# MadrMan/gpgpuraytrace

Measured on AMD Instinct MI355X. Metric: Mray/s + ms/frame at 1920×1080, 1/2/4/8 MI355X; % HBM roofline, higher is better.
Workload: dtype f32

## Files before the change

### gpgpuraytrace_amd/csrc/rt_kernels.hip

```cpp
#include <hip/hip_runtime.h>

#include <cstdio>
#include <cstdlib>
#include <type_traits>

#include "rt_kernels.h"
#include "rt_shader.h"
#include "rt_variants.h"

using namespace rts;
using rtm::f3;

namespace {

constexpr int kPermWords = 128 * 128;
constexpr int kNpOct = RT_NP_OCTAVES + 3;
constexpr int kOctWords = kNpOct * 4;
constexpr int kOctBase = (int)kLdsGz / 4 + (int)(kLdsGz - kLdsGxy) / 4;
constexpr int kNoiseLdsWords = kOctBase + kOctWords;
static_assert(kNoiseLdsWords % 4 == 0, "LDS carved after the noise image stays 16-byte aligned");
static_assert(kLdsGxy == (uint32_t)kPermWords * 4u, "gxy follows the perm2D texels");

__device__ __forceinline__ void load_noise_lds(uint32_t* lds, const uint32_t* __restrict__ perm2d,
                                               const float4* __restrict__ grad, const RtConsts* __restrict__ k)
// ... 100 lines not shown

template <bool STATS, int BS, int LPR>
__global__ void __launch_bounds__(BS) k_camerarays_group(const RtConsts* __restrict__ k,
                                                          const uint32_t* __restrict__ perm2d,
                                                          const float4* __restrict__ grad, float4* __restrict__ out,
                                                          RtStats* stats, const FrameTable* __restrict__ ft)
{
    constexpr int L = RT_NOMADPLAINS;
    if (ft) out = ft->cam[blockIdx.y];
    __shared__ __attribute__((aligned(16))) uint32_t lds[kNoiseLdsWords];
    load_noise_lds(lds, perm2d, grad, k);
    const int i = blockIdx.x * (BS / LPR) + (int)(threadIdx.x / LPR);
    if (i >= RT_CAMERA_RES * RT_CAMERA_RES) return;
    Ctx c = make_ctx(k, lds);
    if (ft) c = frame_ctx_cam(c, ft, blockIdx.y);
    const uint32_t j = threadIdx.x & (LPR - 1u), base = threadIdx.x & 63u & ~(LPR - 1u);
    const SegOctaves<LPR> g = seg_octaves<LPR>(c, j);
    int tx = i % RT_CAMERA_RES, ty = i / RT_CAMERA_RES;
    const float r31 = rtm::rcp(31.0f);
    uint32_t pxs = (uint32_t)(((float)tx * r31) * k->screen[0]);
    uint32_t pys = (uint32_t)(((float)ty * r31) * k->screen[1]);
    f3 p, dir;
    get_pixel_ray(c, (float)pxs, (float)pys, &p, &dir);
    March<L, false> st;
    march_begin(c, st, p, RT_CAMERA_NEAR, 2.0f, dir);
    uint32_t noise = 0;
    while (march_live<L, false, true>(c, st, RT_CAMERA_FAR, 0)) {
        auto dens = [&](f3 q) {
            uint32_t used;
            float d = density_nomadplains_seg<LPR>(c, g, q, j, base, &used);
            noise += used + 1u;
            return d;
        };
        march_step_with<L, false, true, decltype(dens), true>(c, st, dens);
    }
    RayResult rr = march_result(st);
    if (rr.density < 0.0f) rr.pd.w = RT_CAMERA_FAR;
    if (j == 0) {
        out[i] = make_float4(rr.pd.x, rr.pd.y, rr.pd.z, rr.pd.w);
        if constexpr (STATS) {
            atomicAdd(&stats->prepass_steps, (unsigned long long)rr.steps);
            atomicAdd(&stats->noise_calls, (unsigned long long)noise);
        }
    }
}

template <class Depth>
__device__ __forceinline__ float cd_get_depth(Depth depth, int x, int y)
{
    x = x < 0 ? 0 : (x >= RT_CAMERA_RES ? RT_CAMERA_RES - 1 : x);
    y = y < 0 ? 0 : (y >= RT_CAMERA_RES ? RT_CAMERA_RES - 1 : y);
    return depth(x, y);
}
template <class Depth>
__device__ __forceinline__ float cd_interp(Depth d, int x, int y)
{
    if (x < 0) {
        float m = cd_get_depth(d, x + 1, y);
        float dd = cd_get_depth(d, x + 2, y) - m;
        return m - dd;
    }
    if (x >= RT_CAMERA_RES) {
        float m = cd_get_depth(d, x - 1, y);
        float dd = cd_get_depth(d, x - 2, y) - m;
        return m - dd;
    }
    if (y < 0) {
// ... 980 lines not shown
                live = true;
            }
            __builtin_amdgcn_s_waitcnt(0);
            if (lane == 0) {
                q.l_head = head + take;
                q.ls_top = sl - more;
            }
            q_unlock(&q.lock, lane);
            const uint32_t lid = late(lane);
            const uint32_t j = lid & (LPR - 1u), base = lid & ~(LPR - 1u);
            const SegOctaves<LPR> g = seg_octaves<LPR>(c, j);
            for (;;) {
                if (live && !march_live<L, true, true>(cl, st, aux_ao(aux) ? RT_AO_END : 100.0f, 0)) {
                    if (j == 0u) {
                        stat(aux_ao(aux) ? BlockStats::AO : BlockStats::SHADOW, (uint32_t)st.iters);
                        if (kAoSlots > 0u && aux_ao_slot(aux)) ao_slot_finish(st, t, aux);
                        else long_finish<L>(k, m, s_fr, fin, finp, samples, aocc, t, aux, st);
                    }
                    live = false;
                }
                if (!__ballot(live)) break;
                WT(wt[25]++;)
                if (live) {
                    auto dens = [&](f3 q0) {
                        uint32_t used;
                        const float d = density_nomadplains_seg<LPR>(cl, g, q0, j, base, &used);
                        if constexpr (STATS) {
                            if (j == 0u) atomicAdd(&s_st.v[BlockStats::NOISE], (unsigned long long)(used + 1u));
                            if (lane == (uint32_t)__builtin_ctzll(__ballot(1)))
                                atomicAdd(&s_st.v[BlockStats::NOISE_WAVES], (unsigned long long)SegOctaves<LPR>::R);
                        }
                        return d;
                    };
                    march_step_with<L, true, true, decltype(dens), true>(cl, st, dens);
                }
            }
            uint32_t fa = j == 0u ? aux : kAuxAO;
            if (__ballot(fa < kFinSlots || aux_slot_free(fa))) {
                q_lock(&q.lock, lane);
                free_fin_locked(false, fa);
                q_unlock(&q.lock, lane);
            }
        }
    };

    auto primary_seg = [&](const Ctx& cf, March<L, true>& st, bool lv, uint64_t lb, float spx, float spy) {
        if constexpr (L == RT_NOMADPLAINS && kPrimarySeg > 0u && (!STATS || kStatsPrimarySeg)) {
            constexpr uint32_t LPR = 64u / (kPrimarySeg ? kPrimarySeg : 8u);
            const uint32_t lid = late(lane);
            const uint32_t j = lid & (LPR - 1u), grp = lid / LPR, base = lid & ~(LPR - 1u);
            const uint32_t n = (uint32_t)__popcll(lb);
            uint32_t src = lid;
            uint64_t rem = lb;
            for (uint32_t r = 0; r < n; ++r) {
                const uint32_t sl = (uint32_t)__builtin_ctzll(rem);
                rem &= rem - 1ull;
                src = grp == r ? sl : src;
            }
            March<L, true> sg;
            sg.p = rtm::mk(__shfl(st.p.x, (int)src), __shfl(st.p.y, (int)src), __shfl(st.p.z, (int)src));
            sg.dir = rtm::mk(__shfl(st.dir.x, (int)src), __shfl(st.dir.y, (int)src), __shfl(st.dir.z, (int)src));
            sg.sd = __shfl(st.sd, (int)src);
            sg.dist = __shfl(st.dist, (int)src);
            sg.step = __shfl(st.step, (int)src);
            sg.lastStep = __shfl(st.lastStep, (int)src);
            sg.d = __shfl(st.d, (int)src);
            sg.iters = __shfl(st.iters, (int)src);
            sg.f = {0.0f, 0.0f, 0.0f, 0.0f};
            sg.fog = false;
            bool live = grp < n;
            const SegOctaves<LPR> g = seg_octaves<LPR>(cf, j);
            for (;;) {
                if (live && !march_live<L, true, false>(cf, sg, RT_CAMERA_FAR, max_steps)) live = false;
                if (!__ballot(live)) break;
                if (live) {
                    auto dens = [&](f3 q0) {
                        uint32_t used;
                        const float d = density_nomadplains_seg<LPR, true>(cf, g, q0, j, base, &used);
                        if constexpr (STATS) {
                            if (j == 0u) atomicAdd(&s_st.v[BlockStats::NOISE], (unsigned long long)(used + 1u));
                            if (lane == (uint32_t)__builtin_ctzll(__ballot(1)))
                                atomicAdd(&s_st.v[BlockStats::NOISE_WAVES], (unsigned long long)SegOctaves<LPR>::R);
                        }
                        return d;
                    };
                    march_step_with<L, true, false, decltype(dens), true>(cf, sg, dens);
                }
            }
            const int back = (int)(lane_rank(lb) * LPR);
            const float sd = __shfl(sg.sd, back), dist = __shfl(sg.dist, back), step = __shfl(sg.step, back);
            const float last = __shfl(sg.lastStep, back), d = __shfl(sg.d, back);
            const int iters = __shfl(sg.iters, back);
            if (lv) {
                st.sd = sd;
                st.dist = dist;
                st.step = step;
                st.lastStep = last;
                st.d = d;
                st.iters = iters;
            }
            f3 p, dir;
            get_pixel_ray(cf, spx, spy, &p, &dir);
            st.p = p;
            st.dir = rtm::scale(dir, rtm::rcp(rtm::length(dir)));
        }
    };

    auto do_shade = [&]() {
        q_lock(&q.lock, lane);
        const uint32_t top = vload(q.h_top);
        const uint32_t take = top < 64u ? top : 64u;
        float4 r0 = make_float4(0.0f, 0.0f, 0.0f, 0.0f), r1 = r0, r2 = r0;
        if (lane < take) {
            const uint32_t ri = (top - take + lane) * HR;
            r0 = ld_rec(hq, ri);
            if constexpr (HR == 3u) {
                r1 = ld_rec(hq, ri + 1u);
                r2 = ld_rec(hq, ri + 2u);
            }
// ... 78 lines not shown
            push_long(valid, ao, t, ao_aux);
        }
    };

    auto do_prepass = [&](const FrameTable* __restrict__ pft, uint32_t qt, bool own) {
        if constexpr (L == RT_NOMADPLAINS) {
            constexpr uint32_t LPR = RT_PREPASS_LPR, RPW = 64u / LPR;
            constexpr uint32_t WPF = RT_CAMERA_RES * RT_CAMERA_RES / RPW;
            const uint32_t f = qt / WPF;
            const uint32_t ray0 = (qt - f * WPF) * RPW;
            const uint32_t ray = ray0 + late(lane) / LPR;
            const uint32_t lid = late(lane);
            const uint32_t j = lid & (LPR - 1u), base = lid & ~(LPR - 1u);
            Ctx cp = c;
            cp.k = pft->kcam[0];
            cp.kf = (KPtr)pft->kcam[f];
            cp.eye = rtm::mk(uniform_f(cp.kf->eye[0]), uniform_f(cp.kf->eye[1]), uniform_f(cp.kf->eye[2]));
            cp.sun = rtm::mk(uniform_f(cp.kf->sun[0]), uniform_f(cp.kf->sun[1]), uniform_f(cp.kf->sun[2]));
            const uint32_t tx = ray % RT_CAMERA_RES, ty = ray / RT_CAMERA_RES;
            const float r31 = rtm::rcp(31.0f);
            const uint32_t pxs = (uint32_t)(((float)tx * r31) * cp.k->screen[0]);
            const uint32_t pys = (uint32_t)(((float)ty * r31) * cp.k->screen[1]);
            f3 p, dir;
            get_pixel_ray(cp, (float)pxs, (float)pys, &p, &dir);
            March<L, false> st;
            march_begin(cp, st, p, RT_CAMERA_NEAR, 2.0f, dir);
            const SegOctaves<LPR> g = seg_octaves<LPR>(cp, j);
            __builtin_amdgcn_s_setprio(RT_FUSE_PRIO);
            while (march_live<L, false, true>(cp, st, RT_CAMERA_FAR, 0)) {
                auto dens = [&](f3 q0) {
                    uint32_t used;
                    return density_nomadplains_seg<LPR, false>(cp, g, q0, j, base, &used);
                };
                march_step_with<L, false, true, decltype(dens), true>(cp, st, dens);
            }
            __builtin_amdgcn_s_setprio(0);
            RayResult rr = march_result(st);
            if (rr.density < 0.0f) rr.pd.w = RT_CAMERA_FAR;
            if (j == 0u) {
                typedef float v4f __attribute__((ext_vector_type(4)));
                const v4f v = {rr.pd.x, rr.pd.y, rr.pd.z, rr.pd.w};
                float4* dst = pft->cam[f] + ray;
                asm volatile("global_store_dwordx4 %0, %1, off sc1" : : "v"(dst), "v"(v) : "memory");
            }
            asm volatile("s_waitcnt vmcnt(0)" : : : "memory");
            if (!own) {
                if (lane == 0) __hip_atomic_fetch_add(np.ctl + 1, RPW, __ATOMIC_RELAXED, __HIP_MEMORY_SCOPE_AGENT);
                return;
            }
            typedef uint32_t __attribute__((address_space(1))) guint;
            guint* gf = (guint*)(gp.gate + f * RT_GATE_WORDS);
            uint32_t old = 0;
            if (lane == 0) {
                const uint32_t task = ray0 / RT_FUSE_RAYS_PER_TASK;
                bool whole = true;
                if constexpr (RPW < RT_FUSE_RAYS_PER_TASK)
                    whole = __hip_atomic_fetch_add(gf + RT_GATE_TASKS + task, RPW, __ATOMIC_RELAXED,
                                                   __HIP_MEMORY_SCOPE_AGENT) == RT_FUSE_RAYS_PER_TASK - RPW;
                if (whole) {
                    __hip_atomic_fetch_or(gf + (task >> 5), 1u << (task & 31u), __ATOMIC_RELAXED, __HIP_MEMORY_SCOPE_AGENT);
                    old = __hip_atomic_fetch_add(gf + RT_GATE_CTR, (uint32_t)RT_FUSE_RAYS_PER_TASK, __ATOMIC_RELAXED,
                                                 __HIP_MEMORY_SCOPE_AGENT);
                }
            }
            if ((uint32_t)__builtin_amdgcn_readfirstlane(old) == RT_CAMERA_RES * RT_CAMERA_RES - RT_FUSE_RAYS_PER_TASK) {
                if (gp.debug & 2u) {
                    const uint64_t t0 = __builtin_amdgcn_s_memrealtime();
// ... 122 lines not shown
        }
        Ctx cf = frame_ctx(c, ft, f);
        cf.nz.phase = RT_PHASE_PRIMARY;
        uint32_t px, py;
        const bool valid = unit_pixel(m, f, u, lane, W, H, &px, &py);
        const float pxf = (float)px, pyf = (float)py;
        float plane_x = 0.0f;
        if (valid) {
            float spx = pxf * k->rcp_w, spy = pyf * k->rcp_h;
            const uint32_t cell = (uint32_t)rtm::fma(rtm::floor(spy * 32.0f), 32.0f, rtm::floor(spx * 32.0f));
            if (GATED && !cells_in) {
                const float4* cam = ft->cam[f];
                plane_x = cell_bracket([&](int x, int y) { return cam_depth_sc1(cam, x, y); }, (int)(cell % RT_CAMERA_RES),
                                       (int)(cell / RT_CAMERA_RES)).x;
            } else if (GATED) {
                typedef const float __attribute__((address_space(1))) gcfloat;
                plane_x = __hip_atomic_load((gcfloat*)(ft->cells[f] + cell), __ATOMIC_RELAXED, __HIP_MEMORY_SCOPE_AGENT);
            } else {
                plane_x = gptr(ft->cells[f])[cell].x;
            }
        }
        for (uint32_t a = 0; a < aa; ++a) {
            const uint32_t t = f * m.frame_samples + (u * 64u + lane) * aa + a;
            March<L, true> st;
            st.d = 0.0f;
            bool lv = false;
            if (valid) {
                f3 p, dir;
                get_pixel_ray(cf, pxf + k->aa_off[a][0], pyf + k->aa_off[a][1], &p, &dir);
                march_begin(cf, st, p, plane_x, 1.0f, dir);
                lv = true;
            }
            __builtin_amdgcn_s_setprio(0);
            for (uint32_t it = 0;; ++it) {
                lv = lv && march_live<L, true, false>(cf, st, RT_CAMERA_FAR, max_steps);
                const uint64_t lb = __ballot(lv);
                if (lb == 0ull) break;
                RT_DIAG_LIVE_HIST(if (lane == (uint32_t)__builtin_ctzll(__ballot(1))) atomicAdd(&g_live_hist[__popcll(lb)], 1ull);)
                RT_DIAG_PRIMARY_STEPS(if (lv) {
                    cf.nz.phase = RT_COUNT_PHASE;
                    count_noise(cf.nz);
                    cf.nz.phase = RT_PHASE_PRIMARY;
                })
                if constexpr (L == RT_NOMADPLAINS && kPrimarySeg > 0u && (!STATS || kStatsPrimarySeg)) {
                    if ((uint32_t)__popcll(lb) <= kPrimarySeg) {
                        primary_seg(cf, st, lv, lb, pxf + k->aa_off[a][0], pyf + k->aa_off[a][1]);
                        break;
                    }
                }
#if RT_FBM_EXIT
                if constexpr (L == RT_NOMADPLAINS) {
                    if (lv) {
                        const float ns = st.step * k->step_factor;
                        const bool allow = st.dist + ns < RT_CAMERA_FAR && ns > k->min_limit &&
                                           !(max_steps > 0 && st.iters + 1 >= max_steps);
                        march_step_with<L, true, false>(cf, st, [&](f3 q) { return density_nomadplains_x(cf, q, allow); });
                    }
                } else
#endif
                if (lv) march_step<L, true, false>(cf, st);
                if (it == 96u) __builtin_amdgcn_s_setprio(1);
                else if (it == 224u) __builtin_amdgcn_s_setprio(2);
                else if (it == 384u) __builtin_amdgcn_s_setprio(3);
            }
            __builtin_amdgcn_s_setprio(0);
            const bool hit = valid && st.d > 0.0f;
            WT(if (valid) wp_maxit = max(wp_maxit, (uint32_t)st.iters);)
            RayResult rr;
            if (valid) {
                rr = march_result(st);
                stat(BlockStats::PRIMARY, (uint32_t)st.iters);
                if (!hit) {
                    const float4 v = miss_sample(cf, pxf + k->aa_off[a][0], pyf + k->aa_off[a][1], rr.pd.w, rr.fc);
                    if (aa == 1u) {
                        const uint32_t px8 = unorm8(v.x) | (unorm8(v.y) << 8) | (unorm8(v.z) << 16) | 0xff000000u;
                        if (m.packed) {
                            if (!(RT_DIAG_SKIP & 1)) gptr(ft->out8[f])[packed_index(late(u * 64u + lane))] = px8;
                        } else {
                            const size_t o = (size_t)py * W + px;
                            if (!(RT_DIAG_SKIP & 1)) gptr(ft->out8[f])[o] = px8;
                            if (float4* o32 = ft->out32[f]) gstore(o32 + o, make_float4(v.x, v.y, v.z, 1.0f));
                        }
                    } else {
                        samples[t] = v;
                    }
                }
            }
            const uint64_t hb = __ballot(hit);
            if (lane == 0) hitmask[(f * m.n_units + u) * aa + a] = (m.fit || m.fitm) ? 0ull : hb;
            if (hb) {
                const uint32_t n = (uint32_t)__popcll(hb), rank = lane_rank(hb);
                if (hit) stat(BlockStats::HITS, 1u);
                q_lock(&q.lock, lane);
                const uint32_t top = vload(q.h_top);
                const bool fits = (uint32_t)__builtin_amdgcn_readfirstlane(top) + n <= hit_cap;
                if (hit && fits) hit_store<L>(hq + (size_t)(top + rank) * HR, t, rr);
// ... 428 lines not shown
                                                   uint32_t* __restrict__ steps, uint32_t i)
{
    RayResult rr = march_result(st);
    if (rr.density < 0.0f) rr.pd.w = RT_CAMERA_FAR;
    gstore(out + i, make_float4(rr.pd.x, rr.pd.y, rr.pd.z, rr.pd.w));
    if constexpr (STEPS) steps[i] = (uint32_t)st.iters;
}

template <bool STEPS, int BS, int LPR>
__global__ void __launch_bounds__(BS) k_rayquery_seg(const RtConsts* __restrict__ k,
                                                      const uint32_t* __restrict__ perm2d,
                                                      const float4* __restrict__ grad,
                                                      const float4* __restrict__ rays, float4* __restrict__ out,
                                                      uint32_t* __restrict__ steps, uint32_t n, float ex, float ey,
                                                      float ez)
{
    constexpr int L = RT_NOMADPLAINS;
    __shared__ __attribute__((aligned(16))) uint32_t lds[kNoiseLdsWords];
    load_noise_lds(lds, perm2d, grad, k);
    const uint32_t i = blockIdx.x * (uint32_t)(BS / LPR) + threadIdx.x / (uint32_t)LPR;
    if (i >= n) return;
    Ctx c = make_ctx(k, lds);
    c.eye = rtm::mk(ex, ey, ez);
    const uint32_t j = threadIdx.x & (LPR - 1u), base = threadIdx.x & 63u & ~(LPR - 1u);
    const SegOctaves<LPR> g = seg_octaves<LPR>(c, j);
    const QueryRay r = load_query_ray(rays, i);
    March<L, false> st;
    march_begin(c, st, r.p, RT_CAMERA_NEAR, 2.0f, r.dir);
    while (march_live<L, false, true>(c, st, RT_CAMERA_FAR, 0)) {
        auto dens = [&](f3 q) {
            uint32_t used;
            return density_nomadplains_seg<LPR>(c, g, q, j, base, &used);
        };
        march_step_with<L, false, true, decltype(dens), true>(c, st, dens);
    }
    if (j == 0) store_query_result<STEPS>(st, out, steps, i);
}

template <int L, bool STEPS>
__global__ void __launch_bounds__(1024) k_rayquery(const RtConsts* __restrict__ k, const uint32_t* __restrict__ perm2d,
                                                   const float4* __restrict__ grad, const float4* __restrict__ rays,
                                                   float4* __restrict__ out, uint32_t* __restrict__ steps, uint32_t n,
                                                   float ex, float ey, float ez, uint32_t* __restrict__ counter,
                                                   uint32_t refill_live)
{
#ifdef RT_RAYQ_UTIL
    uint32_t util_wave = 0, util_lane = 0;
#endif
    __shared__ __attribute__((aligned(16))) uint32_t lds[kNoiseLdsWords];
    load_noise_lds(lds, perm2d, grad, k);
    Ctx c = make_ctx(k, lds);
    c.eye = rtm::mk(ex, ey, ez);
    const uint32_t lane = threadIdx.x & 63u;
    March<L, false> st{};
    uint32_t idx = 0;
    bool has = false, live = false;
    bool more = true;
    for (;;) {
        uint64_t lv = __ballot(live);
        if (more && (uint32_t)__popcll(lv) <= refill_live) {
            const uint32_t cnt = 64u - (uint32_t)__popcll(lv);
            const uint32_t first = wave_fetch(counter, lane, cnt);
            if (!live) {
                if (has) store_query_result<STEPS>(st, out, steps, idx);
                idx = first + lane_rank(~lv);
                has = idx < n;
                if (has) {
// ... 77 lines not shown

__global__ void k_debug_math(int op, const float* __restrict__ a, const float* __restrict__ b, float* __restrict__ y,
                             int n)
{
    int i = blockIdx.x * blockDim.x + threadIdx.x;
    if (i >= n) return;
    if (op == 12) {
        const float d2 = rtm::fbits(rtm::bits(a[0]) + (uint32_t)i);
        bool near;
        const int est = rts::np_octaves_estimate(d2, &near);
        uint32_t* cnt = reinterpret_cast<uint32_t*>(y);
        if (!near && est != rts::np_octaves_exact(d2)) atomicAdd(&cnt[0], 1u);
        const uint64_t bn = __ballot(near), ba = __ballot(true);
        if (__lane_id() == 0) {
            if (bn) atomicAdd(&cnt[1], (uint32_t)__popcll(bn));
            atomicAdd(&cnt[2], (uint32_t)__popcll(ba));
        }
        return;
    }
    float x = a[i], v = 0.0f;
    switch (op) {
    case 0: v = rtm::exp2(x); break;
    case 1: v = rtm::log2(x); break;
    case 2: v = rtm::exp(x); break;
    case 3: v = rtm::sin(x); break;
    case 4: v = rtm::cos(x); break;
    case 5: v = rtm::sqrt(x); break;
    case 6: v = rtm::rcp(x); break;
    case 7: v = rtm::rcp(rtm::sqrt(x)); break;
    case 8: v = rtm::pow(x, b[i]); break;
    case 9: v = rtm::max(x, b[i]); break;
    case 10: v = rtm::min(x, b[i]); break;
    case 11: v = rtm::pow_nonneg(x, b[i]); break;
    default: v = 0.0f; break;
    }
    y[i] = v;
}

template <int L>
__global__ void __launch_bounds__(256) k_debug_noise(const RtConsts* __restrict__ k, const uint32_t* __restrict__ perm2d,
                                                     const float4* __restrict__ grad, const float* __restrict__ xyz,
                                                     float* __restrict__ out, int n, int density)
{
    __shared__ __attribute__((aligned(16))) uint32_t lds[kNoiseLdsWords];
    load_noise_lds(lds, perm2d, grad, k);
    int i = blockIdx.x * blockDim.x + threadIdx.x;
    if (i >= n) return;
    Ctx c = make_ctx(k, lds);
    f3 p = rtm::mk(xyz[3 * i], xyz[3 * i + 1], xyz[3 * i + 2]);
    if (density == 2) {
        out[i] = noise3d_z0(c.nz, p.x, p.y);
    } else {
        out[i] = density ? get_density<L>(c, p) : noise3d(c.nz, p.x, p.y, p.z);
    }
}

__global__ void __launch_bounds__(256) k_debug_sky(const RtConsts* __restrict__ k, const uint32_t* __restrict__ perm2d,
                                                   const float4* __restrict__ grad, const float* __restrict__ dirs,
                                                   float* __restrict__ out, int n)
{
    __shared__ __attribute__((aligned(16))) uint32_t lds[kNoiseLdsWords];
    load_noise_lds(lds, perm2d, grad, k);
    int i = blockIdx.x * blockDim.x + threadIdx.x;
    if (i >= n) return;
    Ctx c = make_ctx(k, lds);
    const f3 d = rtm::mk(dirs[3 * i], dirs[3 * i + 1], dirs[3 * i + 2]);
    const SkyColor sc = get_rayleigh_mie(c, d);
    const float space = get_space_color(c, d);
    float* o = out + 7 * i;
    o[0] = sc.mie.x;
    o[1] = sc.mie.y;
    o[2] = sc.mie.z;
    o[3] = sc.rayleigh.x;
    o[4] = sc.rayleigh.y;
    o[5] = sc.rayleigh.z;
    o[6] = space;
}

__global__ void __launch_bounds__(64) k_debug_spin(const unsigned long long* base, unsigned long long until_ticks,
                                                  unsigned long long ticks, unsigned long long* stamp)
{
    const unsigned long long t0 = __builtin_amdgcn_s_memrealtime();
    if (stamp && threadIdx.x == 0) *stamp = t0;
    const unsigned long long ready = base ? base[0] + until_ticks : t0;
// ... 69 lines not shown
```

### gpgpuraytrace_amd/csrc/rt_math.h

```cpp
#pragma once

#include <stdint.h>
#include <string.h>

#if defined(__HIPCC__)
#include <hip/hip_runtime.h>
#define RT_HD __host__ __device__ __forceinline__
#else
#include <math.h>
#define RT_HD static inline
#endif

namespace rtm {

RT_HD float fma(float a, float b, float c) { return __builtin_fmaf(a, b, c); }

RT_HD uint32_t bits(float f)
{
#if defined(__HIP_DEVICE_COMPILE__)
    return __builtin_bit_cast(uint32_t, f);
#else
    uint32_t u;
    memcpy(&u, &f, 4);
    return u;
// ... 117 lines not shown
        mb -= 0x00800000u;
        e += 1;
    }
    float f = fbits(mb) - 1.0f;
    float p = -0x1.c362c0p-4f;
    p = fma(p, f, 0x1.7d9132p-3f);
    p = fma(p, f, -0x1.87381ap-3f);
    p = fma(p, f, 0x1.a2f85ep-3f);
    p = fma(p, f, -0x1.eabd64p-3f);
    p = fma(p, f, 0x1.277e9ap-2f);
    p = fma(p, f, -0x1.715a76p-2f);
    p = fma(p, f, 0x1.ec7094p-2f);
    p = fma(p, f, -0x1.715470p-1f);
    p = fma(p, f, 0x1.715476p+0f);
    return fma(f, p, (float)e);
}

RT_HD float exp2_fin(float x)
{
    if (x < -150.0f) return 0.0f;
    if (x >= 128.0f) return __builtin_inff();
    float n = rint(x);
    float f = x - n;
    float p = 0x1.41a6fep-13f;
    p = fma(p, f, 0x1.5f44f0p-10f);
    p = fma(p, f, 0x1.3b2dfep-7f);
    p = fma(p, f, 0x1.c6aed6p-5f);
    p = fma(p, f, 0x1.ebfbdap-3f);
    p = fma(p, f, 0x1.62e430p-1f);
    p = fma(p, f, 1.0f);
    return __builtin_ldexpf(p, (int)n);
}

RT_HD float pow_nonneg_flat(float x, float y)
{
#if !defined(__HIP_DEVICE_COMPILE__)
    return exp2_fin(y * log2_nonneg(x));
#else
    int e;
    float m = __builtin_frexpf(x, &e);
    uint32_t mb = bits(m) + 0x00800000u;
    e -= 1;
    const bool hi = mb > 0x3fb504f3u;
    mb = hi ? mb - 0x00800000u : mb;
    e = hi ? e + 1 : e;
    float f = fbits(mb) - 1.0f;
    float p = -0x1.c362c0p-4f;
    p = fma(p, f, 0x1.7d9132p-3f);
    p = fma(p, f, -0x1.87381ap-3f);
    p = fma(p, f, 0x1.a2f85ep-3f);
    p = fma(p, f, -0x1.eabd64p-3f);
    p = fma(p, f, 0x1.277e9ap-2f);
    p = fma(p, f, -0x1.715a76p-2f);
    p = fma(p, f, 0x1.ec7094p-2f);
    p = fma(p, f, -0x1.715470p-1f);
    p = fma(p, f, 0x1.715476p+0f);
    const float lg = x == 0.0f ? -__builtin_inff() : fma(f, p, (float)e);
    const float a = y * lg;
    const float ac = min(max(a, -150.0f), 128.0f);
    const float n = rint(ac);
    const float g = ac - n;
    float q = 0x1.41a6fep-13f;
    q = fma(q, g, 0x1.5f44f0p-10f);
    q = fma(q, g, 0x1.3b2dfep-7f);
    q = fma(q, g, 0x1.c6aed6p-5f);
    q = fma(q, g, 0x1.ebfbdap-3f);
    q = fma(q, g, 0x1.62e430p-1f);
    q = fma(q, g, 1.0f);
    float r = __builtin_ldexpf(q, (int)n);
    r = a >= 128.0f ? __builtin_inff() : r;
    return a < -150.0f ? 0.0f : r;
#endif
}

RT_HD float pow(float x, float y) { return exp2(y * log2(x)); }
RT_HD float pow_nonneg(float x, float y) { return exp2_fin(y * log2_nonneg(x)); }
RT_HD float exp(float x) { return exp2(x * 0x1.715476p+0f); }
RT_HD float exp_fin(float x) { return exp2_fin(x * 0x1.715476p+0f); }

RT_HD void sincos(float x, float* s, float* c)
{
    float k = rint(x * 0x1.45f306p-1f);
    float r = fma(-k, 0x1.921fb6p+0f, x);
    r = fma(-k, -0x1.777a5cp-25f, r);
    r = fma(-k, -0x1.000000p-49f, r);
    float u = r * r;
    float ps = fma(fma(-0x1.99071ap-13f, u, 0x1.110630p-7f), u, -0x1.555540p-3f);
    float sv = fma(r * u, ps, r);
    float pc = fma(fma(fma(0x1.9906cap-16f, u, -0x1.6c0786p-10f), u, 0x1.55553ap-5f), u, -0.5f);
    float cv = fma(u, pc, 1.0f);
    int q = (int)(k - 4.0f * floor(k * 0.25f));
    float so = (q & 1) ? cv : sv;
    float co = (q & 1) ? sv : cv;
    if (q == 2 || q == 3) so = -so;
    if (q == 1 || q == 2) co = -co;
    *s = so;
    *c = co;
}
RT_HD float sin(float x)
{
    if (isnan_(x) || abs(x) == __builtin_inff()) return __builtin_nanf("");
    float s, c;
    sincos(x, &s, &c);
    return s;
// ... 28 lines not shown
```

### gpgpuraytrace_amd/csrc/rt_shader.h

```cpp
#pragma once

#include "rt_math.h"
#include "rt_types.h"
#include "rt_variants.h"

namespace rts {

using rtm::f3;
using rtm::fma;

constexpr uint32_t kLdsGxy = 0x10000u, kLdsGz = 0x18000u;
typedef float v2f __attribute__((ext_vector_type(2)));

struct NoiseView {
    const char* img;
    const float4* oct;
    uint32_t so16;
    mutable uint64_t calls;
    __attribute__((address_space(3))) unsigned long long* lds_calls;
    uint32_t phase;
};
enum { RT_PHASE_OTHER = 0, RT_PHASE_PRIMARY = 1, RT_PHASE_LONG = 2, RT_PHASE_SHADE = 3 };

__device__ __forceinline__ void count_noise(const NoiseView& nz)
// ... 95 lines not shown
}

template <bool FAST = false>
__device__ __forceinline__ NoiseCell noise3d_cell(const NoiseView& nz, float px, float py, float pz)
{
    NoiseCell c;
    const float fx = rtm::floor(px), fy = rtm::floor(py), fz = rtm::floor(pz);
    c.xy = v2(px, py) - v2(fx, fy);
    c.z = pz - fz;
    c.Z = layer_index<FAST>(fz);
    c.t = *reinterpret_cast<const uint32_t*>(nz.img + texel_offset<FAST>(fx, fy));
    return c;
}

__device__ __forceinline__ float noise3d_finish(const NoiseView& nz, const NoiseCell& c)
{
    const v2f uxy = fade2(c.xy);
    const v2f xy1 = c.xy + v2(-1.0f, -1.0f);
    return noise3d_lattice(nz, c.t, c.Z, c.xy.x, c.xy.y, xy1.x, xy1.y, c.z, uxy.x, uxy.y, fade(c.z));
}

__device__ __forceinline__ float noise3d_raw(const NoiseView& nz, float px, float py, float pz)
{
    return noise3d_finish(nz, noise3d_cell(nz, px, py, pz));
}

template <bool FAST = false>
__device__ __forceinline__ float noise3d_z0(const NoiseView& nz, float px, float py)
{
    const float fx = rtm::floor(px), fy = rtm::floor(py);
    const v2f xy = v2(px, py) - v2(fx, fy);
    const v2f uxy = fade2(xy);
    const v2f xy1 = xy + v2(-1.0f, -1.0f);
    const uint32_t w = *reinterpret_cast<const uint32_t*>(nz.img + texel_offset<FAST>(fx, fy)) & 0x7f7f7f7fu;
    auto g_at = [&](uint32_t sel) {
        return *reinterpret_cast<const float4*>(nz.img + __builtin_amdgcn_perm(w, nz.so16, sel));
    };
    const float4 a0 = g_at(0x0c020400u), a1 = g_at(0x0c020500u), b0 = g_at(0x0c020600u), b1 = g_at(0x0c020700u);
    const float x = xy.x, y = xy.y, x1 = xy1.x, y1 = xy1.y;
    const float g00 = fma(a0.z, y, a0.x * x), g10 = fma(b0.z, y, b0.x * x1);
    const float g01 = fma(a1.z, y1, a1.x * x), g11 = fma(b1.z, y1, b1.x * x1);
    const float lx0 = fma(uxy.x, g10 - g00, g00), lx1 = fma(uxy.x, g11 - g01, g01);
    return fma(uxy.y, lx1 - lx0, lx0);
}

__device__ __forceinline__ float noise3d(const NoiseView& nz, float px, float py, float pz)
{
    count_noise(nz);
    return noise3d_raw(nz, px, py, pz);
}

typedef const __attribute__((address_space(4))) RtConsts* KPtr;

struct Ctx {
    NoiseView nz;
    const RtConsts* k;
    KPtr kf;
    f3 eye;
    f3 sun;
};

constexpr float kOctEps = 1.0f / 2048.0f;

__device__ __forceinline__ int np_octaves_exact(float d2)
{
    const float dist = rtm::max(rtm::sqrt(d2), 0.01f);
    return (int)rtm::max(18.0f - rtm::pow_nonneg(dist, 0.33f), 2.0f);
}

__device__ __forceinline__ int np_octaves_estimate(float d2, bool* near)
{
// ... 60 lines not shown
    asm volatile("" : "+v"(op));
    const uint32_t oe = op + (uint32_t)n_oct * 16u;
    #pragma unroll 1
    do {
        const v4f oc = *(lds_f4*)(uintptr_t)op;
        count_noise(c.nz);
        s = fma(noise3d_finish(c.nz, noise3d_cell<FAST>(c.nz, q0.x * oc.x, q0.y * oc.y, q0.z * oc.x)), oc.z, s);
        op += 16u;
        asm("" : "+v"(op));
    } while (op != oe);
#else
    #pragma unroll 1
    for (int N = 1; N <= RT_NP_OCTAVES + RT_EXTRA_OCTAVE; ++N) {
        if (N > n_oct + RT_EXTRA_OCTAVE) break;
        const float4 oc = c.nz.oct[N];
        count_noise(c.nz);
        s = fma(noise3d_finish(c.nz, noise3d_cell<FAST>(c.nz, q0.x * oc.x, q0.y * oc.y, q0.z * oc.x)),
                N <= n_oct ? oc.z : 0.0f, s);
    }
#endif
    return s;
}

__device__ __forceinline__ float density_nomadplains(const Ctx& c, f3 p)
{
    float d = -p.y;
    f3 p1 = rtm::scale(p, 0.4f);
    float s = 0.0f;
    f3 q0 = rtm::scale(p1, 0.006f);
    const int n_oct = np_octaves(c, p);
    const float qm = rtm::max(rtm::max(rtm::abs(q0.x), rtm::abs(q0.y)), rtm::abs(q0.z));
    const bool fast = !__ballot(!(qm * c.nz.oct[n_oct].x < kFastCellRange));
    s = fast ? np_fbm<true>(c, q0, n_oct) : np_fbm<false>(c, q0, n_oct);
    s = rtm::pow_nonneg(rtm::abs(fma(s, 30.0f, 1.0f)) * 35.0f, c.k->np_expo);
    count_noise(c.nz);
    const float sn = fast ? noise3d_z0<true>(c.nz, p1.x * 0.007138f, p1.z * 0.007138f)
                          : noise3d_z0<false>(c.nz, p1.x * 0.007138f, p1.z * 0.007138f);
    float steep = rtm::sat((sn - 0.2f) * 6.0f) * 7.5f;
    s = terraces(s, p1.y, steep);
    const float lb = rtm::sat((-p1.y + 10.0f) * 1.6f);
    s = fma(__ballot(lb != 0.0f) ? rtm::pow_nonneg(lb, 1.5f) : 0.0f, 19.0f, s);
    return d + s;
}

#if RT_FBM_EXIT
constexpr float kNoiseBound = 1.05f;
template <bool FAST>
__device__ __forceinline__ float fbm_range(const Ctx& c, f3 q0, uint32_t op, uint32_t oe, float s)
{
    typedef float v4f __attribute__((ext_vector_type(4)));
    typedef __attribute__((address_space(3))) const volatile v4f lds_f4;
    #pragma unroll 1
    do {
        const v4f oc = *(lds_f4*)(uintptr_t)op;
        count_noise(c.nz);
        s = fma(noise3d_finish(c.nz, noise3d_cell<FAST>(c.nz, q0.x * oc.x, q0.y * oc.y, q0.z * oc.x)), oc.z, s);
        op += 16u;
        asm("" : "+v"(op));
    } while (op != oe);
    return s;
}
__device__ __forceinline__ float density_nomadplains_x(const Ctx& c, f3 p, bool allow)
{
    constexpr int K = RT_FBM_EXIT;
    float d = -p.y;
    f3 p1 = rtm::scale(p, 0.4f);
    f3 q0 = rtm::scale(p1, 0.006f);
    const int n_oct = np_octaves(c, p);
    const float qm = rtm::max(rtm::max(rtm::abs(q0.x), rtm::abs(q0.y)), rtm::abs(q0.z));
    const bool fast = !__ballot(!(qm * c.nz.oct[n_oct].x < kFastCellRange));
    count_noise(c.nz);
    const float sn = fast ? noise3d_z0<true>(c.nz, p1.x * 0.007138f, p1.z * 0.007138f)
                          : noise3d_z0<false>(c.nz, p1.x * 0.007138f, p1.z * 0.007138f);
    const float steep = rtm::sat((sn - 0.2f) * 6.0f) * 7.5f;
// ... 109 lines not shown
            }
            float nx = q0.x * sx, ny = q0.y * sy, nzz = q0.z * sx;
            if (r == 0 && v == 0u) {
                nx = p1.x * 0.007138f;
                ny = p1.z * 0.007138f;
                nzz = 0.0f;
            }
            n = noise3d_raw(c.nz, nx, ny, nzz);
        }
        nv[r] = need ? n : 0.0f;
    }
    float s = 0.0f, on0;
    constexpr bool kDpp = RT_SEG_DPP && LPR <= 16;
    if constexpr (kDpp) {
        s = seg_chain_dpp<LPR, 1>(nv, g.rcp, s);
        on0 = nv[0];
    } else if constexpr (LOWREG) {
#pragma unroll
        for (int N = 1; N <= RT_NP_OCTAVES; ++N) {
            int idx = (int)(base + (uint32_t)(N % LPR));
            asm volatile("" : "+v"(idx) : "v"(s));
            s = fma(__shfl(nv[N / LPR], idx, 64), g.rcp[N], s);
        }
        on0 = __shfl(nv[0], (int)base, 64);
    } else {
        float on[NV];
#pragma unroll
        for (int v = 0; v < NV; ++v) on[v] = __shfl(nv[v / LPR], (int)(base + (uint32_t)(v % LPR)), 64);
#pragma unroll
        for (int N = 1; N <= RT_NP_OCTAVES; ++N) s = fma(on[N], g.rcp[N], s);
        on0 = on[0];
    }
    *octaves = (uint32_t)n_oct;
    s = rtm::pow_nonneg_flat(rtm::abs(fma(s, 30.0f, 1.0f)) * 35.0f, c.k->np_expo);
    float steep = rtm::sat((on0 - 0.2f) * 6.0f) * 7.5f;
    s = terraces(s, p1.y, steep);
    const float lb = rtm::sat((-p1.y + 10.0f) * 1.6f);
    const float lift = __ballot(lb != 0.0f) ? rtm::pow_nonneg_flat(lb, 1.5f) : 0.0f;
    s = fma(lift, 19.0f, s);
    if constexpr (kDpp) return seg_bcast<LPR>(d + s);
    return d + s;
}

__device__ __forceinline__ float density_testing(const Ctx&, f3 p)
{
    float d = -p.y;
    return fma(rtm::sin(p.x * 0.1f) * rtm::cos(p.z * 0.1f), 10.0f, d);
}

__device__ __forceinline__ float density_simple(const Ctx& c, f3 p)
{
    float d = -p.y;
    f3 q = rtm::scale(p, 0.006f);
    float n = noise3d(c.nz, q.x * 1.0f, q.y * 0.0f, q.z * 1.0f) * 150.0f;
    asm volatile("" : "+v"(p.x), "+v"(p.y), "+v"(p.z) : "v"(n));
    f3 q2 = rtm::scale(p, 0.002f);
    float w2 = rtm::min(rtm::max(fma(-p.y, 1.5f, 50.0f), 0.0f), 36.0f);
    n = fma(-fma(noise3d(c.nz, q2.x, q2.y, q2.z), 0.5f, 0.5f), w2, n);
    asm volatile("" : "+v"(p.x), "+v"(p.y), "+v"(p.z) : "v"(n));
    f3 q3 = rtm::scale(p, 0.003f);
    float w3 = rtm::min(rtm::max(fma(-p.y, 1.5f, 10.0f), 0.0f), 36.0f);
    n = fma(-fma(noise3d(c.nz, q3.x, q3.y, q3.z), 0.5f, 0.5f), w3, n);
    asm volatile("" : "+v"(p.x), "+v"(p.y), "+v"(p.z) : "v"(n));
    f3 q4 = rtm::scale(p, 0.06f);
    float S = c.k->np_scale[1];
    n = fma(noise3d(c.nz, q4.x * S, q4.y * c.k->np_scale_y[1], q4.z * S), c.k->np_rcp[1], n);
    return d + n;
}

__device__ __forceinline__ float density_greenrocks(const Ctx& c, f3 p)
{
// ... 93 lines not shown
{
    m.fog = fog;
    const RtConsts* k = c.k;
    m.f = {0.0f, 0.0f, 0.0f, 0.0f};
    m.d = 0.0f;
    float dirLength = rtm::length(dir);
    m.step = fma(-dist, k->one_minus_step_factor, (0.03f * stepmod) * dirLength);
    m.lastStep = m.step;
    float il = rtm::rcp(dirLength);
    dir = rtm::scale(dir, il);
    if constexpr (March<L, CALCFOG>::FOG) if (fog) {
        float hd = dist * 0.5f;
        f3 mp = rtm::mk(fma(dir.x * dist, 0.5f, p.x), fma(dir.y * dist, 0.5f, p.y), fma(dir.z * dist, 0.5f, p.z));
        f4 mf = get_fog<L>(c, mp, hd);
        m.f.x = fma(mf.x, dist, m.f.x);
        m.f.y = fma(mf.y, dist, m.f.y);
        m.f.z = fma(mf.z, dist, m.f.z);
        m.f.w = fma(mf.w, dist, m.f.w);
    }
    m.p = p;
    m.dir = dir;
    m.dist = dist;
    m.sd = 0.0f;
    m.iters = 0;
}

template <int L, bool CALCFOG, bool SKIPREFINE>
__device__ __forceinline__ bool march_live(const Ctx& c, const March<L, CALCFOG>& m, float enddist, int max_steps)
{
    if (SKIPREFINE && m.d > 0.0f) return false;
    return m.dist < enddist && m.step > c.k->min_limit && !(max_steps > 0 && m.iters >= max_steps);
}

template <int L, bool CALCFOG, bool SKIPREFINE, class Density, bool FLAT = false>
__device__ __forceinline__ void march_step_with(const Ctx& c, March<L, CALCFOG>& m, Density density)
{
    const RtConsts* k = c.k;
    ++m.iters;
    const f3 rayp = rtm::mk(fma(m.dir.x, m.dist, m.p.x), fma(m.dir.y, m.dist, m.p.y), fma(m.dir.z, m.dist, m.p.z));
    m.sd = m.dist;
    m.d = density(rayp);
    f4 fs = {0.0f, 0.0f, 0.0f, 0.0f};
    if constexpr (March<L, CALCFOG>::FOG) if (m.fog) {
        f4 g = get_fog<L>(c, rayp, m.dist);
        fs.x = g.x * m.step;
        fs.y = g.y * m.step;
        fs.z = g.z * m.step;
        fs.w = g.w * m.step;
    }
    constexpr bool kFog = March<L, CALCFOG>::FOG;
    if (m.d > 0.0f) {
        if constexpr (SKIPREFINE) return;
        m.dist = m.dist - m.lastStep;
        m.step = m.step * 0.3f;
        if constexpr (kFog) {
            m.f.x = m.f.x - fs.x;
            m.f.y = m.f.y - fs.y;
            m.f.z = m.f.z - fs.z;
            m.f.w = m.f.w - fs.w;
        }
    } else {
        const float sx = rtm::abs(rtm::min(m.d + 5.0f, 0.0f));
        float stepmult;
        if constexpr (FLAT) stepmult = 1.0f + (__ballot(sx != 0.0f) ? rtm::pow_nonneg_flat(sx, k->density_factor) : 0.0f);
        else stepmult = 1.0f + rtm::pow_nonneg(sx, k->density_factor);
        m.step = m.step * k->step_factor;
        m.lastStep = m.step * stepmult;
        m.dist = m.dist + m.lastStep;
        if constexpr (kFog) {
            m.f.x = m.f.x + fs.x;
            m.f.y = m.f.y + fs.y;
            m.f.z = m.f.z + fs.z;
            m.f.w = m.f.w + fs.w;
        }
    }
}

template <int L, bool CALCFOG, bool SKIPREFINE>
__device__ __forceinline__ void march_step(const Ctx& c, March<L, CALCFOG>& m)
{
    march_step_with<L, CALCFOG, SKIPREFINE>(c, m, [&](f3 q) { return get_density<L>(c, q); });
}

template <int L, bool CALCFOG>
__device__ __forceinline__ RayResult march_result(const March<L, CALCFOG>& m)
{
    RayResult rr;
    const bool stepped = m.iters > 0;
    rr.pd.x = stepped ? fma(m.dir.x, m.sd, m.p.x) : 0.0f;
    rr.pd.y = stepped ? fma(m.dir.y, m.sd, m.p.y) : 0.0f;
    rr.pd.z = stepped ? fma(m.dir.z, m.sd, m.p.z) : 0.0f;
    rr.sd = m.sd;
    rr.pd.w = m.dist;
    rr.fc = m.f;
    rr.density = m.d;
    rr.steps = (float)m.iters;
    return rr;
}
// ... 235 lines not shown
```

Baseline: 1509.

## Use wave-uniform pow everywhere, restructure primary march loop, load only needed gradient components

```diff
diff --git a/gpgpuraytrace_amd/csrc/rt_kernels.hip b/gpgpuraytrace_amd/csrc/rt_kernels.hip
--- a/gpgpuraytrace_amd/csrc/rt_kernels.hip
+++ b/gpgpuraytrace_amd/csrc/rt_kernels.hip
@@ -156,7 +156,7 @@
             noise += used + 1u;
             return d;
         };
-        march_step_with<L, false, true, decltype(dens), true>(c, st, dens);
+        march_step_with<L, false, true>(c, st, dens);
     }
     RayResult rr = march_result(st);
     if (rr.density < 0.0f) rr.pd.w = RT_CAMERA_FAR;
@@ -1203,7 +1203,7 @@
                         }
                         return d;
                     };
-                    march_step_with<L, true, true, decltype(dens), true>(cl, st, dens);
+                    march_step_with<L, true, true>(cl, st, dens);
                 }
             }
             uint32_t fa = j == 0u ? aux : kAuxAO;
@@ -1255,7 +1255,7 @@
                         }
                         return d;
                     };
-                    march_step_with<L, true, false, decltype(dens), true>(cf, sg, dens);
+                    march_step_with<L, true, false>(cf, sg, dens);
                 }
             }
             const int back = (int)(lane_rank(lb) * LPR);
@@ -1400,7 +1400,7 @@
                     uint32_t used;
                     return density_nomadplains_seg<LPR, false>(cp, g, q0, j, base, &used);
                 };
-                march_step_with<L, false, true, decltype(dens), true>(cp, st, dens);
+                march_step_with<L, false, true>(cp, st, dens);
             }
             __builtin_amdgcn_s_setprio(0);
             RayResult rr = march_result(st);
@@ -1589,36 +1589,36 @@
                 lv = true;
             }
             __builtin_amdgcn_s_setprio(0);
-            for (uint32_t it = 0;; ++it) {
-                lv = lv && march_live<L, true, false>(cf, st, RT_CAMERA_FAR, max_steps);
-                const uint64_t lb = __ballot(lv);
-                if (lb == 0ull) break;
-                RT_DIAG_LIVE_HIST(if (lane == (uint32_t)__builtin_ctzll(__ballot(1))) atomicAdd(&g_live_hist[__popcll(lb)], 1ull);)
-                RT_DIAG_PRIMARY_STEPS(if (lv) {
+            uint32_t it = 0;
+            while (lv) {
+                lv = march_live<L, true, false>(cf, st, RT_CAMERA_FAR, max_steps);
+                if (!lv) break;
+                [[maybe_unused]] const uint64_t lb = __ballot(1);
+                RT_DIAG_LIVE_HIST(if (lane == (uint32_t)__builtin_ctzll(lb)) atomicAdd(&g_live_hist[__popcll(lb)], 1ull);)
+                RT_DIAG_PRIMARY_STEPS({
                     cf.nz.phase = RT_COUNT_PHASE;
                     count_noise(cf.nz);
                     cf.nz.phase = RT_PHASE_PRIMARY;
                 })
                 if constexpr (L == RT_NOMADPLAINS && kPrimarySeg > 0u && (!STATS || kStatsPrimarySeg)) {
-                    if ((uint32_t)__popcll(lb) <= kPrimarySeg) {
-                        primary_seg(cf, st, lv, lb, pxf + k->aa_off[a][0], pyf + k->aa_off[a][1]);
-                        break;
-                    }
+                    if ((uint32_t)__popcll(lb) <= kPrimarySeg) break;
                 }
 #if RT_FBM_EXIT
                 if constexpr (L == RT_NOMADPLAINS) {
-                    if (lv) {
-                        const float ns = st.step * k->step_factor;
-                        const bool allow = st.dist + ns < RT_CAMERA_FAR && ns > k->min_limit &&
-                                           !(max_steps > 0 && st.iters + 1 >= max_steps);
-                        march_step_with<L, true, false>(cf, st, [&](f3 q) { return density_nomadplains_x(cf, q, allow); });
-                    }
+                    const float ns = st.step * k->step_factor;
+                    const bool allow = st.dist + ns < RT_CAMERA_FAR && ns > k->min_limit &&
+                                       !(max_steps > 0 && st.iters + 1 >= max_steps);
+                    march_step_with<L, true, false>(cf, st, [&](f3 q) { return density_nomadplains_x(cf, q, allow); });
                 } else
 #endif
-                if (lv) march_step<L, true, false>(cf, st);
+                march_step<L, true, false>(cf, st);
                 if (it == 96u) __builtin_amdgcn_s_setprio(1);
                 else if (it == 224u) __builtin_amdgcn_s_setprio(2);
                 else if (it == 384u) __builtin_amdgcn_s_setprio(3);
+                ++it;
+            }
+            if constexpr (L == RT_NOMADPLAINS && kPrimarySeg > 0u && (!STATS || kStatsPrimarySeg)) {
+                if (const uint64_t lb = __ballot(lv)) primary_seg(cf, st, lv, lb, pxf + k->aa_off[a][0], pyf + k->aa_off[a][1]);
             }
             __builtin_amdgcn_s_setprio(0);
             const bool hit = valid && st.d > 0.0f;
@@ -2113,7 +2113,7 @@
             uint32_t used;
             return density_nomadplains_seg<LPR>(c, g, q, j, base, &used);
         };
-        march_step_with<L, false, true, decltype(dens), true>(c, st, dens);
+        march_step_with<L, false, true>(c, st, dens);
     }
     if (j == 0) store_query_result<STEPS>(st, out, steps, i);
 }
@@ -2257,6 +2257,7 @@
     case 9: v = rtm::max(x, b[i]); break;
     case 10: v = rtm::min(x, b[i]); break;
     case 11: v = rtm::pow_nonneg(x, b[i]); break;
+    case 13: v = rtm::pow_nonneg_wave(x, b[i]); break;
     default: v = 0.0f; break;
     }
     y[i] = v;
@@ -2275,6 +2276,8 @@
     f3 p = rtm::mk(xyz[3 * i], xyz[3 * i + 1], xyz[3 * i + 2]);
     if (density == 2) {
         out[i] = noise3d_z0(c.nz, p.x, p.y);
+    } else if (density == 3) {
+        out[i] = noise3d_z0<true>(c.nz, p.x, p.y);
     } else {
         out[i] = density ? get_density<L>(c, p) : noise3d(c.nz, p.x, p.y, p.z);
     }
diff --git a/gpgpuraytrace_amd/csrc/rt_math.h b/gpgpuraytrace_amd/csrc/rt_math.h
--- a/gpgpuraytrace_amd/csrc/rt_math.h
+++ b/gpgpuraytrace_amd/csrc/rt_math.h
@@ -173,7 +173,7 @@
     return __builtin_ldexpf(p, (int)n);
 }
 
-RT_HD float pow_nonneg_flat(float x, float y)
+RT_HD float pow_nonneg_wave(float x, float y)
 {
 #if !defined(__HIP_DEVICE_COMPILE__)
     return exp2_fin(y * log2_nonneg(x));
@@ -196,11 +196,15 @@
     p = fma(p, f, 0x1.ec7094p-2f);
     p = fma(p, f, -0x1.715470p-1f);
     p = fma(p, f, 0x1.715476p+0f);
-    const float lg = x == 0.0f ? -__builtin_inff() : fma(f, p, (float)e);
-    const float a = y * lg;
-    const float ac = min(max(a, -150.0f), 128.0f);
-    const float n = rint(ac);
-    const float g = ac - n;
+    const float a = y * fma(f, p, (float)e);
+    const bool special = (__ballot(!(a >= -150.0f)) | __ballot(a >= 128.0f)) != 0ull;
+    float n = rint(a);
+    float g = a - n;
+    if (__builtin_expect(special, false)) {
+        const float ac = __builtin_amdgcn_fmed3f(a, -150.0f, 128.0f);
+        n = rint(ac);
+        g = ac - n;
+    }
     float q = 0x1.41a6fep-13f;
     q = fma(q, g, 0x1.5f44f0p-10f);
     q = fma(q, g, 0x1.3b2dfep-7f);
@@ -208,9 +212,8 @@
     q = fma(q, g, 0x1.ebfbdap-3f);
     q = fma(q, g, 0x1.62e430p-1f);
     q = fma(q, g, 1.0f);
-    float r = __builtin_ldexpf(q, (int)n);
-    r = a >= 128.0f ? __builtin_inff() : r;
-    return a < -150.0f ? 0.0f : r;
+    const float r = __builtin_ldexpf(q, (int)n);
+    return x == 0.0f ? 0.0f : r;
 #endif
 }
 
diff --git a/gpgpuraytrace_amd/csrc/rt_shader.h b/gpgpuraytrace_amd/csrc/rt_shader.h
--- a/gpgpuraytrace_amd/csrc/rt_shader.h
+++ b/gpgpuraytrace_amd/csrc/rt_shader.h
@@ -151,11 +151,23 @@
     const v2f xy = v2(px, py) - v2(fx, fy);
     const v2f uxy = fade2(xy);
     const v2f xy1 = xy + v2(-1.0f, -1.0f);
-    const uint32_t w = *reinterpret_cast<const uint32_t*>(nz.img + texel_offset<FAST>(fx, fy)) & 0x7f7f7f7fu;
+    uint32_t to;
+    if constexpr (FAST) {
+        const uint32_t mx4 = rtm::bits(fma(fx, 4.0f, kMagic)), my9 = rtm::bits(fma(fy, 512.0f, kMagic));
+        to = (mx4 & 0x1fcu) | (my9 & 0xfe00u);
+    } else {
+        to = texel_offset<false>(fx, fy);
+    }
+    const uint32_t w = *reinterpret_cast<const uint32_t*>(nz.img + to) & 0x7f7f7f7fu;
+    typedef __attribute__((address_space(3))) const volatile float lds_f;
+    struct G2 {
+        float x, z;
+    };
     auto g_at = [&](uint32_t sel) {
-        return *reinterpret_cast<const float4*>(nz.img + __builtin_amdgcn_perm(w, nz.so16, sel));
+        lds_f* g = (lds_f*)(nz.img + __builtin_amdgcn_perm(w, nz.so16, sel));
+        return G2{g[0], g[2]};
     };
-    const float4 a0 = g_at(0x0c020400u), a1 = g_at(0x0c020500u), b0 = g_at(0x0c020600u), b1 = g_at(0x0c020700u);
+    const G2 a0 = g_at(0x0c020400u), a1 = g_at(0x0c020500u), b0 = g_at(0x0c020600u), b1 = g_at(0x0c020700u);
     const float x = xy.x, y = xy.y, x1 = xy1.x, y1 = xy1.y;
     const float g00 = fma(a0.z, y, a0.x * x), g10 = fma(b0.z, y, b0.x * x1);
     const float g01 = fma(a1.z, y1, a1.x * x), g11 = fma(b1.z, y1, b1.x * x1);
@@ -282,14 +294,14 @@
     const float qm = rtm::max(rtm::max(rtm::abs(q0.x), rtm::abs(q0.y)), rtm::abs(q0.z));
     const bool fast = !__ballot(!(qm * c.nz.oct[n_oct].x < kFastCellRange));
     s = fast ? np_fbm<true>(c, q0, n_oct) : np_fbm<false>(c, q0, n_oct);
-    s = rtm::pow_nonneg(rtm::abs(fma(s, 30.0f, 1.0f)) * 35.0f, c.k->np_expo);
+    s = rtm::pow_nonneg_wave(rtm::abs(fma(s, 30.0f, 1.0f)) * 35.0f, c.k->np_expo);
     count_noise(c.nz);
     const float sn = fast ? noise3d_z0<true>(c.nz, p1.x * 0.007138f, p1.z * 0.007138f)
                           : noise3d_z0<false>(c.nz, p1.x * 0.007138f, p1.z * 0.007138f);
     float steep = rtm::sat((sn - 0.2f) * 6.0f) * 7.5f;
     s = terraces(s, p1.y, steep);
     const float lb = rtm::sat((-p1.y + 10.0f) * 1.6f);
-    s = fma(__ballot(lb != 0.0f) ? rtm::pow_nonneg(lb, 1.5f) : 0.0f, 19.0f, s);
+    s = fma(__ballot(lb != 0.0f) ? rtm::pow_nonneg_wave(lb, 1.5f) : 0.0f, 19.0f, s);
     return d + s;
 }
 
@@ -465,11 +477,11 @@
         on0 = on[0];
     }
     *octaves = (uint32_t)n_oct;
-    s = rtm::pow_nonneg_flat(rtm::abs(fma(s, 30.0f, 1.0f)) * 35.0f, c.k->np_expo);
+    s = rtm::pow_nonneg_wave(rtm::abs(fma(s, 30.0f, 1.0f)) * 35.0f, c.k->np_expo);
     float steep = rtm::sat((on0 - 0.2f) * 6.0f) * 7.5f;
     s = terraces(s, p1.y, steep);
     const float lb = rtm::sat((-p1.y + 10.0f) * 1.6f);
-    const float lift = __ballot(lb != 0.0f) ? rtm::pow_nonneg_flat(lb, 1.5f) : 0.0f;
+    const float lift = __ballot(lb != 0.0f) ? rtm::pow_nonneg_wave(lb, 1.5f) : 0.0f;
     s = fma(lift, 19.0f, s);
     if constexpr (kDpp) return seg_bcast<LPR>(d + s);
     return d + s;
@@ -629,7 +641,7 @@
     return m.dist < enddist && m.step > c.k->min_limit && !(max_steps > 0 && m.iters >= max_steps);
 }
 
-template <int L, bool CALCFOG, bool SKIPREFINE, class Density, bool FLAT = false>
+template <int L, bool CALCFOG, bool SKIPREFINE, class Density>
 __device__ __forceinline__ void march_step_with(const Ctx& c, March<L, CALCFOG>& m, Density density)
 {
     const RtConsts* k = c.k;
@@ -659,8 +671,7 @@
     } else {
         const float sx = rtm::abs(rtm::min(m.d + 5.0f, 0.0f));
         float stepmult;
-        if constexpr (FLAT) stepmult = 1.0f + (__ballot(sx != 0.0f) ? rtm::pow_nonneg_flat(sx, k->density_factor) : 0.0f);
-        else stepmult = 1.0f + rtm::pow_nonneg(sx, k->density_factor);
+        stepmult = 1.0f + (__ballot(sx != 0.0f) ? rtm::pow_nonneg_wave(sx, k->density_factor) : 0.0f);
         m.step = m.step * k->step_factor;
         m.lastStep = m.step * stepmult;
         m.dist = m.dist + m.lastStep;
```

New measurement: 1527, median of 6. 1.01x the previous value.
